# dohlee/chromoformer

Hardware: AMD Instinct MI355X
Metric: genes/sec training (bsz=64, default config) (higher is better)
Workload: dtype f32

## Files before the change

chromoformer_amd/_lib.py:

```python
from __future__ import annotations

import ctypes as C
import os
import subprocess

_HERE = os.path.dirname(os.path.abspath(__file__))
LIB_PATH = os.environ.get("CF_LIB_PATH") or os.path.join(_HERE, "libchromoformer_hip.so")
FLAGS_PATH = LIB_PATH + ".flags"
CSRC = os.path.join(_HERE, "csrc")
MAX_RES = 3
BUCKET_REG, BUCKET_PE = 1, 2
BUCKET_REG_HI, BUCKET_REG_LO = 4, 8
PART_REG_HI, PART_REG_LO = 8, 16


class cf_config(C.Structure):
    _fields_ = [
        ("n_feats", C.c_int), ("d_emb", C.c_int), ("d_head", C.c_int), ("n_out", C.c_int), ("n_res", C.c_int),
        ("binsizes", C.c_int * MAX_RES), ("n_bins", C.c_int * MAX_RES), ("i_max", C.c_int),
        ("embed_layers", C.c_int), ("embed_heads", C.c_int), ("embed_dmodel", C.c_int), ("embed_dff", C.c_int),
        ("pair_layers", C.c_int), ("pair_heads", C.c_int), ("pair_dmodel", C.c_int), ("pair_dff", C.c_int),
        ("reg_layers", C.c_int), ("reg_heads", C.c_int), ("reg_dmodel", C.c_int), ("reg_dff", C.c_int),
        ("max_batch", C.c_int),
    ]
# ... 105 lines not shown
    "cf_pcre_shapley": (C.c_int, [C.c_void_p, C.POINTER(cf_batch), C.c_void_p, C.c_void_p, C.c_void_p]),
    "cf_pcre_epistasis": (C.c_int, [C.c_void_p, C.POINTER(cf_batch), C.c_void_p, C.c_void_p, C.c_void_p]),
    "cf_integrated_gradients": (C.c_int, [C.c_void_p, C.POINTER(cf_batch), C.POINTER(cf_ig_opts), C.POINTER(cf_input_grads), C.c_void_p,
                                          C.c_void_p, C.c_void_p, C.c_void_p]),
    "cf_integrated_gradients_raw": (C.c_int, [C.c_void_p, C.POINTER(cf_batch), C.POINTER(cf_ig_opts), C.POINTER(cf_input_grads),
                                              C.POINTER(cf_input_grads), C.c_void_p, C.c_void_p, C.c_void_p, C.c_void_p]),
    "cf_perturbation_scan": (C.c_int, [C.c_void_p, C.POINTER(cf_batch), C.POINTER(cf_scan_opts), C.c_void_p, C.c_void_p]),
    "cf_adamw_step": (C.c_int, [C.c_void_p, C.c_float, C.c_float, C.c_float, C.c_float, C.c_float, C.c_longlong, C.c_void_p]),
    "cf_debug_copy": (C.c_int, [C.c_void_p, C.c_char_p, C.c_void_p, C.POINTER(C.c_longlong), C.c_void_p]),
    "cf_debug_names": (C.c_char_p, [C.c_void_p]),
    "cf_reduce_adamw_part": (C.c_int, [C.c_void_p, C.c_int, C.c_int, C.c_float, C.c_float, C.c_float, C.c_float, C.c_float, C.c_longlong, C.c_int,
                                       C.c_void_p]),
    "cf_reduce_opt_part": (C.c_int, [C.c_void_p, C.c_int, C.c_int, C.c_float, C.c_float, C.c_float, C.c_float, C.c_float, C.c_longlong, C.c_int,
                                     C.c_void_p]),
    "cf_rider_arm": (C.c_int, [C.c_void_p, C.c_float, C.c_float, C.c_float, C.c_float, C.c_float, C.c_longlong, C.c_int, C.c_int]),
    "cf_launch_counts": (C.c_int, [C.c_void_p, C.POINTER(C.c_int), C.POINTER(C.c_int), C.POINTER(C.c_int)]),
    "cf_op_linear": (C.c_int, [C.c_void_p, C.c_void_p, C.c_void_p, C.c_void_p, C.c_int, C.c_int, C.c_int, C.c_int, C.c_void_p]),
    "cf_op_wgrad": (C.c_int, [C.c_void_p, C.c_void_p, C.c_void_p, C.c_int, C.c_int, C.c_int, C.c_void_p]),
    "cf_op_dgrad": (C.c_int, [C.c_void_p, C.c_void_p, C.c_void_p, C.c_int, C.c_int, C.c_int, C.c_void_p]),
    "cf_bin_regions": (C.c_int, [C.c_void_p, C.c_int, C.c_int, C.c_int, C.c_int, C.c_void_p]),
    "cf_bin_regions_multi": (C.c_int, [C.c_void_p, C.c_int, C.c_int, C.c_int, C.POINTER(C.c_int), C.POINTER(C.c_int), C.c_int, C.c_void_p]),
    "cf_bin_regions_multi_backward": (C.c_int, [C.c_void_p, C.c_int, C.c_int, C.c_int, C.POINTER(C.c_int), C.POINTER(C.c_int), C.c_int, C.c_int,
                                                C.c_void_p]),
    "cf_embed_full": (C.c_int, [C.c_void_p, C.POINTER(cf_batch), C.POINTER(C.c_void_p), C.c_void_p]),
    "cf_gather_batch": (C.c_int, [C.c_void_p, C.POINTER(cf_store), C.c_void_p, C.c_void_p, C.POINTER(cf_batch), C.c_void_p, C.c_void_p]),
    "cf_gather_batch_fwd": (C.c_int, [C.c_void_p, C.POINTER(cf_store), C.c_void_p, C.c_void_p, C.POINTER(cf_batch), C.c_void_p, C.c_void_p]),
    "cf_gather_batch_next": (C.c_int, [C.c_void_p, C.POINTER(cf_store), C.c_void_p, C.c_void_p, C.POINTER(cf_batch), C.c_void_p, C.c_void_p]),
    "cf_gather_batch_only": (C.c_int, [C.c_void_p, C.POINTER(cf_store), C.c_void_p, C.c_void_p, C.POINTER(cf_batch), C.c_void_p, C.c_void_p]),
    "cf_record_step_bwd": (C.c_int, [C.c_void_p, C.c_void_p, C.c_void_p, C.c_void_p, C.c_void_p, C.c_int, C.c_void_p, C.c_void_p, C.c_void_p, C.c_void_p]),
    "cf_record_step": (C.c_int, [C.c_void_p, C.c_void_p, C.c_void_p, C.c_void_p, C.c_void_p, C.c_int, C.c_void_p, C.c_void_p, C.c_void_p, C.c_void_p]),
# ... 104 lines not shown
```

chromoformer_amd/csrc/cf_api.hip:

```cpp
#include "../../include/chromoformer_hip.h"
#include "cf_kernels.h"
#include "cf_input_grad.h"
#include "cf_attn_maps.h"
#include "cf_ablate.h"
#include "cf_coalition.h"
#include "cf_ig.h"
#include "cf_scan.h"
#include "cf_x0_gather.h"

#include <algorithm>
#include <cmath>
#include <cstdarg>
#include <cstdio>
#include <cstdlib>
#include <cstring>
#include <map>
#include <string>
#include <vector>

using namespace cf;

static thread_local std::string g_err;
static int fail(const char* fmt, ...) {
    char buf[512];
// ... 257 lines not shown
    std::vector<WsEntry> ws;
    std::map<std::string, int> ws_index;
    std::string ws_names;
    bool planning = true;
    float *pe[kMaxRes], *pet[kMaxRes];
    float *pe2[kMaxRes], *pet2[kMaxRes];
    bool attc2 = false;
    bool attc1 = true;
    int attc_cap = 64;
    int xcd_map = 1;
    int n_wg_r = 0, n_cs_r = 0;
    long long bucket_split = 0;
    long long bucket_split_hi = 0;
    int n_wg_hi = 0, n_cs_hi = 0;
    int n_wg_short = 0;
    float *featc[kMaxRes], *ex0[kMaxRes], *edx0[kMaxRes], *edout[kMaxRes];
    CentreBuf E[kMaxRes];
    float *xp0[kMaxRes], *dxp0[kMaxRes], *resid[kMaxRes];
    std::vector<CentreBuf> P[kMaxRes];
    std::vector<float*> Rx[kMaxRes], dRx[kMaxRes];
    std::vector<RegBuf> R[kMaxRes];
    float *hin, *h1, *logits, *dlogits, *dh1, *dhin, *loss, *loss_part, *tdbg;
    float* dfreq_part = nullptr;
    bool reg_dfreq_ok = false;
    bool ig_smem_ok = false;
    float* abl_stash[kMaxRes] = {};
    float* abl_freq = nullptr;
    uint8_t* abl_mask[kMaxRes] = {};
    void* abl_mem = nullptr;
    unsigned* coal_tab = nullptr;
// ... 195 lines not shown
            t.k0 = k0;
            t.toff = -1;
            out.push_back(t);
        }
}
static WgJob wg1(const float* A, int lda, const float* B, int ldb, int rpg, float* C, int ldc, int Nn, int Kk) {
    WgJob j;
    memset(&j, 0, sizeof j);
    j.seg[0] = WgSeg{A, B, lda, ldb, rpg};
    j.nseg = 1;
    j.C = C;
    j.ldc = ldc;
    j.Nn = Nn;
    j.Kk = Kk;
    return j;
}
static void push_cs(std::vector<CsTile>& out, const float* src, int ld, int ncols, int rpg, int div, float* dst, const float* src2 = nullptr) {
    for (int c0 = 0; c0 < ncols; c0 += 64) out.push_back(CsTile{src, dst, ld, ncols, c0, rpg, div, src2});
}
static void push_post_cs(std::vector<CsTile>& out, const cf_handle* h, const float* part, int dff, int rpg,
                         const std::string& att_pre, const std::string& ff_pre, int div = kTile) {
    const int kD = h->cfg.d_emb;
    const int pw = post_partial_width(dff, kD);
    push_cs(out, part + 0, pw, kD, rpg, div, h->G_(ff_pre + "ln.weight"));
    push_cs(out, part + kD, pw, kD, rpg, div, h->G_(ff_pre + "ln.bias"));
    push_cs(out, part + 2 * kD, pw, kD, rpg, div, h->G_(ff_pre + "l2.bias"));
    push_cs(out, part + 3 * kD, pw, dff, rpg, div, h->G_(ff_pre + "l1.bias"));
    push_cs(out, part + 3 * kD + dff, pw, kD, rpg, div, h->G_(att_pre + "ln.weight"));
    push_cs(out, part + 4 * kD + dff, pw, kD, rpg, div, h->G_(att_pre + "ln.bias"));
    push_cs(out, part + 5 * kD + dff, pw, kD, rpg, div, h->G_(att_pre + "ff.bias"));
// ... 131 lines not shown
                const float* xin = l == 0 ? b.xin : h->P[r][l - 1].out;
                float* gc = h->G_(lp + "self_att.c_att.weight");
                push_centre_wg(wg, h, b, xin, kD, S, c.pair_dff, h->G_(lp + "self_att.p_att.weight"), gc, gc + (size_t)kD * kD,
                               lp + "self_att.", lp + "ff.", c.pair_heads);
                if (h->trunk) push_post_cs(cs, h, b.partial, c.pair_dff, 1, lp + "self_att.", lp + "ff.", 1);
                else push_post_cs(cs, h, b.partial, c.pair_dff, S, lp + "self_att.", lp + "ff.");
            }
        }
        for (int l = 0; l < c.reg_layers; ++l) {
            std::vector<WgTile>& wgR = l >= c.reg_layers / 2 ? wgHi : wgLo;
            std::vector<CsTile>& csR = l >= c.reg_layers / 2 ? csHi : csLo;
            const std::string lp = fmt("regulation.%d.transformer.layers.%d.", bs, l);
            const RegBuf& b = h->R[r][l];
            const int dff = c.reg_dff;
            const int RDm = c.reg_dmodel, RW = 4 * RDm;
            if (l + 1 == c.reg_layers && h->reg_row0 && h->reg8) {
                float* ga = h->G_(lp + "self_att.att.weight");
                push_wg(wgShort, wg1(b.dqkvg, T * RW, h->Rx[r][l], T * kD, 1, ga, kD, RDm, kD));
                push_wg(wgR, wg1(b.dqkvg + RDm, RW, h->Rx[r][l], kD, T, ga + (size_t)RDm * kD, kD, 2 * RDm, kD));
                push_wg(wgShort, wg1(b.dqkvg + 3 * RDm, T * RW, h->Rx[r][l], T * kD, 1, ga + (size_t)3 * RDm * kD, kD, RDm, kD));
                push_wg(wgShort, wg1(b.dt1, T * kD, b.a, T * RDm, 1, h->G_(lp + "self_att.ff.weight"), RDm, kD, RDm));
                push_wg(wgShort, wg1(b.dpre1, T * dff, b.y1, T * kD, 1, h->G_(lp + "ff.l1.weight"), kD, dff, kD));
                push_wg(wgShort, wg1(b.dt2, T * kD, b.hdn, T * dff, 1, h->G_(lp + "ff.l2.weight"), dff, kD, dff));
            } else {
            push_wg(wgR, wg1(b.dqkvg, RW, h->Rx[r][l], kD, T, h->G_(lp + "self_att.att.weight"), kD, RW, kD));
            push_wg(wgR, wg1(b.dt1, kD, b.a, RDm, T, h->G_(lp + "self_att.ff.weight"), RDm, kD, RDm));
            push_wg(wgR, wg1(b.dpre1, dff, b.y1, kD, T, h->G_(lp + "ff.l1.weight"), kD, dff, kD));
            push_wg(wgR, wg1(b.dt2, kD, b.hdn, dff, T, h->G_(lp + "ff.l2.weight"), dff, kD, dff));
            }
            if (h->reg8) {
                const std::string ap = lp + "self_att.", fp = lp + "ff.";
                push_cs(csR, h->dRx[r][l + 1], kD, kD, T, 1, h->G_(fp + "ln.weight"), b.xh2);
                push_cs(csR, h->dRx[r][l + 1], kD, kD, T, 1, h->G_(fp + "ln.bias"));
                push_cs(csR, b.dt2, kD, kD, T, 1, h->G_(fp + "l2.bias"));
                push_cs(csR, b.dpre1, dff, dff, T, 1, h->G_(fp + "l1.bias"));
                push_cs(csR, b.dy1, kD, kD, T, 1, h->G_(ap + "ln.weight"), b.xh1);
                push_cs(csR, b.dy1, kD, kD, T, 1, h->G_(ap + "ln.bias"));
                push_cs(csR, b.dt1, kD, kD, T, 1, h->G_(ap + "ff.bias"));
            } else {
                push_post_cs(csR, h, b.partial, dff, T, lp + "self_att.", lp + "ff.");
            }
            push_cs(csR, b.dgam, c.reg_heads, c.reg_heads, 1, 1, h->G_(lp + "self_att.gamma_f"));
        }
    }
// ... 56 lines not shown
    wg.insert(wg.begin(), wgHi.begin(), wgHi.end());
    cs.insert(cs.begin(), csLo.begin(), csLo.end());
    cs.insert(cs.begin(), csHi.begin(), csHi.end());
    h->wg_flops_per_gene = 0.0;
    for (const WgTile& t : wg) {
        if (t.n0 || t.k0) continue;
        for (int sgi = 0; sgi < t.nseg; ++sgi) h->wg_flops_per_gene += 2.0 * t.seg[sgi].rows_per_gene * (double)t.Nn * t.Kk;
    }
    if (h->wg_tiles) (void)hipFree(h->wg_tiles);
    if (h->cs_tiles) (void)hipFree(h->cs_tiles);
    h->n_wg = (int)wg.size();
    h->n_cs = (int)cs.size();
    HIP_TRY(hipMalloc(&h->wg_tiles, wg.size() * sizeof(WgTile)));
    HIP_TRY(hipMalloc(&h->cs_tiles, cs.size() * sizeof(CsTile)));
    HIP_TRY(hipMemcpy(h->wg_tiles, wg.data(), wg.size() * sizeof(WgTile), hipMemcpyHostToDevice));
    HIP_TRY(hipMemcpy(h->cs_tiles, cs.data(), cs.size() * sizeof(CsTile), hipMemcpyHostToDevice));
    return 0;
}

extern "C" int cf_abi_version(void) { return CF_ABI_VERSION; }
extern "C" const char* cf_last_error(void) { return g_err.c_str(); }

extern "C" int cf_param_layout(const cf_config* cfg, cf_layout* layout, cf_param_desc* table, int cap) {
    if (!cfg || !layout) return fail("cf_param_layout: null argument");
    std::vector<PDesc> v;
    if (build_layout(*cfg, v, *layout)) return -1;
    if (table) {
        if (cap < (int)v.size()) return fail("cf_param_layout: table capacity %d < %d", cap, (int)v.size());
        for (size_t i = 0; i < v.size(); ++i) {
            cf_param_desc& d = table[i];
            memset(&d, 0, sizeof d);
            snprintf(d.name, sizeof d.name, "%s", v[i].name.c_str());
            d.ndim = v[i].ndim;
            d.shape[0] = v[i].shape[0];
            d.shape[1] = v[i].shape[1];
            d.offset = v[i].offset;
// ... 340 lines not shown
static CentreParams embed_params(const cf_handle* h, int r) {
    const std::string pre = fmt("embed.%d.", h->cfg.binsizes[r]), lp = pre + "transformer.layers.0.";
    const float* att = h->P_(lp + "self_att.att.weight");
    const size_t kD = h->cfg.d_emb;
    return centre_params(h, lp + "self_att.", lp + "ff.", att, att + (size_t)kD * kD, att + (size_t)2 * kD * kD,
                         h->P_(pre + "lin_proj.weight"));
}
static CentreParams pair_params(const cf_handle* h, int r, int l) {
    const std::string pre = fmt("pairwise_interaction.%d.", h->cfg.binsizes[r]), lp = pre + fmt("transformer.layers.%d.", l);
    const float* c_att = h->P_(lp + "self_att.c_att.weight");
    const size_t kD = h->cfg.d_emb;
    return centre_params(h, lp + "self_att.", lp + "ff.", h->P_(lp + "self_att.p_att.weight"), c_att, c_att + (size_t)kD * kD,
                         h->P_(pre + "lin_proj_pcre.weight"));
}

static const void* trunk_kernel(bool bwd, int dff_e, int dff_p, int pair_layers) {
    if (dff_e == 128 && dff_p == 256 && pair_layers == 2) return bwd ? (const void*)k_trunk_bwd<128, 256, 2> : (const void*)k_trunk_fwd<128, 256, 2>;
    return nullptr;
}
static void fill_centre_dev(CentreLayerDev& d, const CentreParams& p, const CentreBuf& b) {
    d.wq_t = p.wq_t, d.wk = p.wk, d.wv_t = p.wv_t, d.wo_t = p.wo_t, d.bo = p.bo, d.g1 = p.g1, d.be1 = p.be1;
    d.w1_t = p.w1_t, d.b1 = p.b1, d.w2_t = p.w2_t, d.b2 = p.b2, d.g2 = p.g2, d.be2 = p.be2;
    d.wq = p.wq, d.wk_t = p.wk_t, d.wv = p.wv, d.wo = p.wo, d.w1 = p.w1, d.w2 = p.w2;
    d.q = b.q, d.qt = b.qt, d.p = b.p, d.w = b.w, d.xbar = b.xbar, d.a = b.a, d.xh1 = b.xh1, d.rs1 = b.rs1, d.y1 = b.y1;
    d.hdn = b.hdn, d.xh2 = b.xh2, d.rs2 = b.rs2, d.out = b.out, d.xin = b.xin;
    d.dt2 = b.dt2, d.dpre1 = b.dpre1, d.dt1 = b.dt1, d.da = b.da, d.dxbar = b.dxbar, d.dqt = b.dqt, d.du = b.du, d.dq = b.dq;
    d.dx = b.dx, d.partial = b.partial;
}
static int build_trunk_table(cf_handle* h) {
    const cf_config& c = h->cfg;
    h->trunk = false;
    if (h->embed_dense || !h->attc2 || c.i_max > kAGMax || c.pair_layers > kMaxPairLayers || kPostWaves != 8) return 0;
    if (c.embed_heads != 2 || c.pair_heads != 2 || c.d_emb != kD) return 0;
    if (!trunk_kernel(false, c.embed_dff, c.pair_dff, c.pair_layers)) return 0;
    if (const char* e = getenv("CF_TRUNK"))
        if (atoi(e) == 0) return 0;
    size_t need = 0;
    for (int r = 0; r < c.n_res; ++r) need = std::max(need, trunk_smem(c.n_bins[r], c.n_feats, std::max(c.embed_dff, c.pair_dff)));
    if (need > 160 * 1024) return 0;
    const size_t need_bwd = std::max(need, (size_t)(kAT / 64) * kWgWaveLds * sizeof(float));
    if (need_bwd > 160 * 1024) return 0;
    if (hipFuncSetAttribute(trunk_kernel(false, c.embed_dff, c.pair_dff, c.pair_layers), hipFuncAttributeMaxDynamicSharedMemorySize, (int)need) != hipSuccess ||
        hipFuncSetAttribute(trunk_kernel(true, c.embed_dff, c.pair_dff, c.pair_layers), hipFuncAttributeMaxDynamicSharedMemorySize, (int)need_bwd) != hipSuccess)
        return 0;
    std::vector<TrunkResDev> tab(c.n_res);
    for (int r = 0; r < c.n_res; ++r) {
        TrunkResDev& t = tab[r];
        memset(&t, 0, sizeof t);
        fill_centre_dev(t.E, embed_params(h, r), h->E[r]);
        for (int l = 0; l < c.pair_layers; ++l) fill_centre_dev(t.P[l], pair_params(h, r, l), h->P[r][l]);
        t.pe = h->pe[r], t.pe2 = h->pe2[r], t.pet2 = h->pet2[r];
        t.wlp_e = embed_params(h, r).wlp;
        t.wlp_p = pair_params(h, r, 0).wlp;
        t.lin_p = h->P_(fmt("pairwise_interaction.%d.lin_proj_p.weight", c.binsizes[r]));
        t.lin_p_t = h->T_(fmt("pairwise_interaction.%d.lin_proj_p.weight", c.binsizes[r]));
// ... 723 lines not shown
            h->pend_record = false;
        }
        ta.lp_jobs = h->lp_jobs;
        ta.rd_tiles = nullptr;
        ta.rd_n = 0;
        ta.rd_batch = B;
        memset(&ta.rd_opt, 0, sizeof ta.rd_opt);
        const bool riding = h->rider.armed;
        if (riding) {
            if (h->capturing) return fail("cf_backward_part: armed riders carry this step's AdamW scalars as launch arguments and cannot be captured");
            ta.rd_n = std::min(h->rider.max_tiles, h->n_wg_r - h->n_wg_short);
            ta.rd_tiles = h->wg_tiles + h->n_wg_short;
            ta.rd_opt = h->rider.o;
        }
        void* kargs[] = {&ta};
        const size_t rider_lds = (size_t)(kAT / 64) * kWgWaveLds * sizeof(float);
        const int rider_rows = ta.rd_n > 0 ? (ta.rd_n + B * (kAT / 64) - 1) / (B * (kAT / 64)) : 0;
        h->time_mark("k_trunk_bwd", st);
        const hipError_t le = hipLaunchKernel(trunk_kernel(true, c.embed_dff, c.pair_dff, c.pair_layers), dim3(B, nres + rider_rows), dim3(kAT), kargs,
                                              ta.rd_n > 0 ? std::max(h->trunk_smem_bytes, rider_lds) : h->trunk_smem_bytes, st);
        h->time_mark("k_trunk_bwd", st);
        ++g_launches;
        if (le != hipSuccess || hipGetLastError() != hipSuccess) {
            return fail("launch k_trunk_bwd failed: %s", hipGetErrorString(le));
        }
        if (riding) {
            h->rider.armed = false;
            h->rider.done = ta.rd_n;
        }
        return 0;
    }
// ... 906 lines not shown
```

chromoformer_amd/csrc/cf_kernels.h:

```cpp
#pragma once
#include <hip/hip_runtime.h>
#include <stdint.h>
#include <type_traits>
#ifndef CF_TRUNK_NT
#define CF_TRUNK_NT 0
#endif

#ifndef CF_TID_OPAQUE
#define CF_TID_OPAQUE 1
#endif
#if CF_TID_OPAQUE
namespace cf {
struct TidProxy {
    struct X {
        __device__ __forceinline__ operator unsigned() const {
            unsigned t = __builtin_amdgcn_workitem_id_x();
            asm volatile("" : "+v"(t));
            return t;
        }
    } x;
    struct Y { __device__ __forceinline__ operator unsigned() const { return __builtin_amdgcn_workitem_id_y(); } } y;
    struct Z { __device__ __forceinline__ operator unsigned() const { return __builtin_amdgcn_workitem_id_z(); } } z;
};
}
// ... 1693 lines not shown
#define CF_OPT_NT 1
#endif
#ifndef CF_RIDER_NT
#define CF_RIDER_NT 0
#endif
#ifndef CF_WG_M
#define CF_WG_M 32
#endif
constexpr int kWgM = CF_WG_M;
constexpr int kWgTk = CF_WG_TK;
constexpr int kWgLdA = 64 + 16;
constexpr int kWgLdB = kWgTk + 4;
__device__ __forceinline__ float4 f4_keep_if(bool keep, const float4& v) {
    return make_float4(keep ? v.x : 0.f, keep ? v.y : 0.f, keep ? v.z : 0.f, keep ? v.w : 0.f);
}
__device__ __forceinline__ bool wg_tile_interior(const WgTile& t) {
    bool ok = t.n0 + 64 <= t.Nn && t.k0 + kWgTk <= t.Kk;
    for (int s = 0; s < t.nseg; ++s) {
        const WgSeg& sg = t.seg[s];
        ok = ok && ((sg.lda | sg.ldb | t.n0 | t.k0) & 3) == 0 && ((reinterpret_cast<uintptr_t>(sg.A) | reinterpret_cast<uintptr_t>(sg.B)) & 15) == 0;
    }
    return ok;
}
template <bool OPT, int D = 1>
__device__ __forceinline__ void wgrad_tile_impl(const WgTile& t, int batch, const AdamFuse* o, float (*As)[kWgM * kWgLdA], float (*Bs)[kWgM * kWgLdB],
                                                const int tid) {
    constexpr int NH = kWgTk / 64;
    const int w = tid >> 6, lane = tid & 63, lr = lane & 15, lq = lane >> 4;
    const int kc = t.k0 + 4 * lr;
    f32x4 acc[4 * NH];
    zero_acc(acc);
// ... 97 lines not shown
                    if (CF_OPT_NT) stg4_nt(o->p + off, pp[i]); else stg4(o->p + off, pp[i]);
                    if (CF_OPT_NT) stg4_nt(o->m + off, mm[i]); else stg4(o->m + off, mm[i]);
                    if (CF_OPT_NT) stg4_nt(o->v + off, vv[i]); else stg4(o->v + off, vv[i]);
                    if (o->keep_grads) stg4(cp, g4);
                    if (o->tiled && t.toff >= 0) {
                        const int ra = t.trow0 + row, k = kc + 64 * h;
                        stg4(o->tiled + t.toff + ((size_t)(ra >> 4) * (t.ldc >> 4) + (k >> 4)) * 256 + (((k & 15) >> 2) * 16 + (ra & 15)) * 4, pp[i]);
                    }
                } else {
                    stg4(cp, g4);
                }
            }
        }
    }
}
constexpr int kWgWaveLds = kWgM * kWgLdA + kWgM * kWgLdB;
template <bool OPT>
__device__ __forceinline__ void wgrad_tile_wave(const WgTile& t, int batch, const AdamFuse* o, float* lds, unsigned long long* stamp = nullptr) {
    static_assert(kWgTk == 64, "one 64 x 64 tile per wave");
    const int lane = threadIdx.x & 63, lr = lane & 15, lq = lane >> 4;
    float* As = lds;
    float* Bs = lds + kWgM * kWgLdA;
    const int kc = t.k0 + 4 * lr;
    f32x4 acc[4][4];
#pragma unroll
    for (int rt = 0; rt < 4; ++rt) zero_acc(acc[rt]);
    const int sm = lane >> 4, sc = (lane & 15) * 4;
    constexpr int NP = kWgM / 4;
    const bool interior = wg_tile_interior(t);
    auto run = [&](auto fast_c) {
        constexpr bool FAST = decltype(fast_c)::value;
        for (int s = 0; s < t.nseg; ++s) {
            const WgSeg sg = t.seg[s];
            const int M = sg.rows_per_gene * batch, nst = (M + kWgM - 1) / kWgM;
            const bool va = ((sg.lda | t.n0) & 3) == 0 && (reinterpret_cast<uintptr_t>(sg.A) & 15) == 0;
            const bool vb = ((sg.ldb | t.k0) & 3) == 0 && (reinterpret_cast<uintptr_t>(sg.B) & 15) == 0;
            float4 ra[NP], rb[NP];
            auto fetch = [&](int st) {
// ... 38 lines not shown
                    for (int rt = 0; rt < 4; ++rt) {
                        const float av = ap[4 * i * kWgLdA + 16 * rt];
                        acc[rt][0] = mfma4(av, bv.x, acc[rt][0]);
                        acc[rt][1] = mfma4(av, bv.y, acc[rt][1]);
                        acc[rt][2] = mfma4(av, bv.z, acc[rt][2]);
                        acc[rt][3] = mfma4(av, bv.w, acc[rt][3]);
                    }
                }
            }
        }
    };
    if (stamp) stamp[0] = __builtin_amdgcn_s_memtime();
    if (interior) run(std::true_type{});
    else run(std::false_type{});
    if (stamp) stamp[1] = __builtin_amdgcn_s_memtime();
    if (kc >= t.Kk) return;
#pragma unroll
    for (int rt = 0; rt < 4; ++rt) {
        float4 pp[4], mm[4], vv[4];
        if (OPT) {
#pragma unroll
            for (int i = 0; i < 4; ++i) {
                const int row = min(t.n0 + rt * 16 + lq * 4 + i, t.Nn - 1);
                const size_t off = (size_t)(t.C + (size_t)row * t.ldc + kc - o->gbase);
                pp[i] = CF_RIDER_NT ? ldg4_nt(o->p + off) : ldg4(o->p + off);
                mm[i] = CF_RIDER_NT ? ldg4_nt(o->m + off) : ldg4(o->m + off);
                vv[i] = CF_RIDER_NT ? ldg4_nt(o->v + off) : ldg4(o->v + off);
            }
            __builtin_amdgcn_sched_barrier(0);
        }
#pragma unroll
        for (int i = 0; i < 4; ++i) {
            const int row = t.n0 + rt * 16 + lq * 4 + i;
            if (row < t.Nn) {
                float* cp = t.C + (size_t)row * t.ldc + kc;
                const float4 g4 = make_float4(acc[rt][0][i], acc[rt][1][i], acc[rt][2][i], acc[rt][3][i]);
                if (OPT) {
                    const size_t off = (size_t)(cp - o->gbase);
                    adamw_elem(pp[i].x, g4.x, mm[i].x, vv[i].x, *o);
                    adamw_elem(pp[i].y, g4.y, mm[i].y, vv[i].y, *o);
                    adamw_elem(pp[i].z, g4.z, mm[i].z, vv[i].z, *o);
                    adamw_elem(pp[i].w, g4.w, mm[i].w, vv[i].w, *o);
                    if (CF_RIDER_NT) stg4_nt(o->p + off, pp[i]); else stg4(o->p + off, pp[i]);
                    if (CF_RIDER_NT) stg4_nt(o->m + off, mm[i]); else stg4(o->m + off, mm[i]);
                    if (CF_RIDER_NT) stg4_nt(o->v + off, vv[i]); else stg4(o->v + off, vv[i]);
                    if (o->keep_grads) stg4(cp, g4);
                } else {
                    stg4(cp, g4);
                }
            }
        }
    }
}
template <bool OPT = false>
__device__ __forceinline__ void wgrad_tile(const WgTile& t, int batch, const AdamFuse* o = nullptr) {
    __shared__ __attribute__((aligned(16))) float As[1][kWgM * kWgLdA];
    __shared__ __attribute__((aligned(16))) float Bs[1][kWgM * kWgLdB];
    wgrad_tile_impl<OPT>(t, batch, o, As, Bs, threadIdx.x);
}

__device__ __forceinline__ int xcd_tile(int b, int n, int on) {
    const int per = (n + 7) >> 3;
    return on ? (b & 7) * per + (b >> 3) : b;
}
__host__ __device__ inline int xcd_grid(int n) { return 8 * ((n + 7) >> 3); }
__global__ __launch_bounds__(256) void k_wgrad(const WgTile* __restrict__ tiles, int n, int batch, int xcd) {
    const int t = xcd_tile(blockIdx.x, n, xcd);
// ... 275 lines not shown
```

chromoformer_amd/csrc/cf_trunk.h:

```cpp
#pragma once

namespace cf {

constexpr int kMaxPairLayers = 4;

struct CentreLayerDev {
    const float *wq_t, *wk, *wv_t, *wo_t, *bo, *g1, *be1, *w1_t, *b1, *w2_t, *b2, *g2, *be2;
    const float *wq, *wk_t, *wv, *wo, *w1, *w2;
    float *q, *qt, *p, *w, *xbar, *a, *xh1, *rs1, *y1, *hdn, *xh2, *rs2, *out, *xin;
    float *dt2, *dpre1, *dt1, *da, *dxbar, *dqt, *du, *dq, *dx, *partial;
};
struct TrunkResDev {
    CentreLayerDev E, P[kMaxPairLayers];
    const float *pe, *pe2, *pet2;
    const float *wlp_e, *wlp_p;
    const float *lin_p_t, *lin_p;
    float *ex0, *featc, *xp0, *dxp0, *edout, *rx0, *drx0;
    float *lp_part_e, *lp_part_p;
    int L, Lpad, LT, pad_;
};
struct TrunkArgs {
    const TrunkResDev* tab;
    const float* pfeats[kMaxRes];
    const uint8_t* pmask[kMaxRes];
// ... 378 lines not shown
    float* const p1 = ldc(&J[1].partial);
    float* out = (job ? p1 : p0) + (size_t)g * (kD * F) + e * F;
#pragma unroll
    for (int k = 0; k < 4; ++k)
        if (fh * 4 + k < F) stg(out + fh * 4 + k, acc[k]);
}

template <int DFF_E, int DFF_P, int PL>
__global__ __launch_bounds__(kAT) void k_trunk_bwd(TrunkArgs a) {
    extern __shared__ __attribute__((aligned(16))) float smem[];
    if ((int)blockIdx.y >= a.n_res) {
        const int w = threadIdx.x >> 6;
        const int t = (((int)blockIdx.y - a.n_res) * gridDim.x + blockIdx.x) * (kAT / 64) + w;
        unsigned long long* stamp = a.tdbg && blockIdx.x == 0 && (int)blockIdx.y == a.n_res && (threadIdx.x & 63) == 0 ? a.tdbg + 64 + 4 * w : nullptr;
        if (stamp) stamp[3] = __builtin_amdgcn_s_memtime();
        if (t < a.rd_n) wgrad_tile_wave<true>(a.rd_tiles[t], a.rd_batch, &a.rd_opt, smem + w * kWgWaveLds, stamp);
        if (stamp) {
            asm volatile("s_waitcnt vmcnt(0)" ::: "memory");
            stamp[2] = __builtin_amdgcn_s_memtime();
        }
        return;
    }
    if (a.rec.cursor && blockIdx.x == 0 && blockIdx.y == 0) record_block(a.rec);
    const int r = a.n_res - 1 - (int)blockIdx.y;
    const TrunkResDev* R = a.tab + r;
    constexpr int DFF_MAX = DFF_E > DFF_P ? DFF_E : DFF_P;
    float* sm = smem;
    float* persist = smem + trunk_scratch_floats(TF(L), DFF_MAX);
    TrunkCtx c{R, a.cfeats[r], a.cmask[r], a.cmstride[r], (int)blockIdx.x, a.S, a.T, a.F, 1, a.scale, a.rscale};
    int stamp_i = 32;
    if (a.tdbg && blockIdx.x == 0 && blockIdx.y == CF_STAMP_Y && threadIdx.x == 0) a.tdbg[stamp_i++] = __builtin_amdgcn_s_memtime();
// ... 37 lines not shown
```

include/chromoformer_hip.h:

```cpp
#ifndef CHROMOFORMER_HIP_H
#define CHROMOFORMER_HIP_H

#include <stddef.h>
#include <stdint.h>

#ifdef __cplusplus
extern "C" {
#endif

#define CF_MAX_RES 3
#define CF_ABI_VERSION 1

typedef struct cf_config {
    int n_feats;
    int d_emb;
    int d_head;
    int n_out;
    int n_res;
    int binsizes[CF_MAX_RES];
    int n_bins[CF_MAX_RES];
    int i_max;
    int embed_layers, embed_heads, embed_dmodel, embed_dff;
    int pair_layers, pair_heads, pair_dmodel, pair_dff;
    int reg_layers, reg_heads, reg_dmodel, reg_dff;
// ... 115 lines not shown
int cf_graph_launch(cf_handle* h, int graph_id, void* stream);

int cf_timing_select(cf_handle* h, const char* kernel);
int cf_timing_read(cf_handle* h, float* total_ms, int* count);
double cf_wgrad_flops(cf_handle* h, int B);
double cf_kernel_flops(cf_handle* h, const char* kernel, int B);
int cf_cu_count(cf_handle* h);
int cf_debug_copy(cf_handle* h, const char* name, float* dst, long long* n_floats, void* stream);
const char* cf_debug_names(cf_handle* h);
int cf_reduce_adamw_part(cf_handle* h, int B, int reduce_buckets, float lr, float beta1, float beta2, float eps,
                         float weight_decay, long long step, int adam_buckets, void* stream);
int cf_reduce_opt_part(cf_handle* h, int B, int bucket, float lr, float beta1, float beta2, float eps, float weight_decay,
                       long long step, int keep_grads, void* stream);
int cf_rider_arm(cf_handle* h, float lr, float beta1, float beta2, float eps, float weight_decay, long long step, int keep_grads,
                 int max_tiles);
int cf_launch_counts(cf_handle* h, int* fwd, int* bwd, int* opt);

int cf_op_linear(const float* A, const float* W, const float* bias, float* C, int M, int N, int K,
                 int relu, void* stream);
int cf_op_wgrad(const float* dY, const float* X, float* dW, int M, int N, int K, void* stream);
int cf_op_dgrad(const float* dY, const float* W, float* dX, int M, int N, int K, void* stream);

typedef struct cf_dense_layer {
    const float *wq, *wkv;
    const float *wo, *bo, *ln1_g, *ln1_b;
    const float *w1, *b1, *w2, *b2, *ln2_g, *ln2_b;
    int d_ff;
} cf_dense_layer;
long long cf_op_dense_layer_workspace(int N, int Lq, int Lk, int d_ff);
int cf_op_dense_layer_fwd(const cf_dense_layer* w, const float* x_q, const float* x_kv, const unsigned char* qvalid,
// ... 105 lines not shown
```

Before: 131,300.

## Share operand panels across eight rider wgrad tiles in one workgroup

Rider weight-gradient tiles in the trunk backward kernel used to run one wave per tile, each staging its own A/B operands in private LDS. When a group of eight consecutive tiles writes the same output matrix with the same segments and sits within a 4x4 panel rectangle, the whole workgroup now cooperatively stages shared A and B panels into double-buffered LDS and each wave computes its tile from them. This cuts redundant global operand loads, at the cost of a larger LDS reservation for the backward kernel and added workgroup-wide synchronisation. A host query, cf_rider_groups, reports how many groups qualify.

Result: no change. 131,100 (-0.2%).

```diff
diff --git a/chromoformer_amd/_lib.py b/chromoformer_amd/_lib.py
--- a/chromoformer_amd/_lib.py
+++ b/chromoformer_amd/_lib.py
@@ -143,6 +143,7 @@
     "cf_reduce_opt_part": (C.c_int, [C.c_void_p, C.c_int, C.c_int, C.c_float, C.c_float, C.c_float, C.c_float, C.c_float, C.c_longlong, C.c_int,
                                      C.c_void_p]),
     "cf_rider_arm": (C.c_int, [C.c_void_p, C.c_float, C.c_float, C.c_float, C.c_float, C.c_float, C.c_longlong, C.c_int, C.c_int]),
+    "cf_rider_groups": (C.c_int, [C.c_void_p, C.POINTER(cf_config), C.c_int, C.c_int, C.POINTER(C.c_int), C.POINTER(C.c_int)]),
     "cf_launch_counts": (C.c_int, [C.c_void_p, C.POINTER(C.c_int), C.POINTER(C.c_int), C.POINTER(C.c_int)]),
     "cf_op_linear": (C.c_int, [C.c_void_p, C.c_void_p, C.c_void_p, C.c_void_p, C.c_int, C.c_int, C.c_int, C.c_int, C.c_void_p]),
     "cf_op_wgrad": (C.c_int, [C.c_void_p, C.c_void_p, C.c_void_p, C.c_int, C.c_int, C.c_int, C.c_void_p]),
diff --git a/chromoformer_amd/csrc/cf_api.hip b/chromoformer_amd/csrc/cf_api.hip
--- a/chromoformer_amd/csrc/cf_api.hip
+++ b/chromoformer_amd/csrc/cf_api.hip
@@ -295,6 +295,7 @@
     long long bucket_split_hi = 0;
     int n_wg_hi = 0, n_cs_hi = 0;
     int n_wg_short = 0;
+    std::vector<WgTile> wg_r_host;
     float *featc[kMaxRes], *ex0[kMaxRes], *edx0[kMaxRes], *edout[kMaxRes];
     CentreBuf E[kMaxRes];
     float *xp0[kMaxRes], *dxp0[kMaxRes], *resid[kMaxRes];
@@ -520,6 +521,27 @@
     j.Nn = Nn;
     j.Kk = Kk;
     return j;
+}
+struct RegWgSrc {
+    const float *dqkvg, *dt1, *a, *dpre1, *y1, *dt2, *hdn, *x;
+    float *g_att, *g_ff, *g_l1, *g_l2;
+};
+static void push_reg_layer_wg(std::vector<WgTile>& wgShort, std::vector<WgTile>& wgR, const cf_config& c, const RegWgSrc& b, bool row0_last) {
+    const int kD = c.d_emb, T = c.i_max + 1, dff = c.reg_dff, RDm = c.reg_dmodel, RW = 4 * RDm;
+    if (row0_last) {
+        float* ga = b.g_att;
+        push_wg(wgShort, wg1(b.dqkvg, T * RW, b.x, T * kD, 1, ga, kD, RDm, kD));
+        push_wg(wgR, wg1(b.dqkvg + RDm, RW, b.x, kD, T, ga + (size_t)RDm * kD, kD, 2 * RDm, kD));
+        push_wg(wgShort, wg1(b.dqkvg + 3 * RDm, T * RW, b.x, T * kD, 1, ga + (size_t)3 * RDm * kD, kD, RDm, kD));
+        push_wg(wgShort, wg1(b.dt1, T * kD, b.a, T * RDm, 1, b.g_ff, RDm, kD, RDm));
+        push_wg(wgShort, wg1(b.dpre1, T * dff, b.y1, T * kD, 1, b.g_l1, kD, dff, kD));
+        push_wg(wgShort, wg1(b.dt2, T * kD, b.hdn, T * dff, 1, b.g_l2, dff, kD, dff));
+    } else {
+        push_wg(wgR, wg1(b.dqkvg, RW, b.x, kD, T, b.g_att, kD, RW, kD));
+        push_wg(wgR, wg1(b.dt1, kD, b.a, RDm, T, b.g_ff, RDm, kD, RDm));
+        push_wg(wgR, wg1(b.dpre1, dff, b.y1, kD, T, b.g_l1, kD, dff, kD));
+        push_wg(wgR, wg1(b.dt2, kD, b.hdn, dff, T, b.g_l2, dff, kD, dff));
+    }
 }
 static void push_cs(std::vector<CsTile>& out, const float* src, int ld, int ncols, int rpg, int div, float* dst, const float* src2 = nullptr) {
     for (int c0 = 0; c0 < ncols; c0 += 64) out.push_back(CsTile{src, dst, ld, ncols, c0, rpg, div, src2});
@@ -681,20 +703,9 @@
             const RegBuf& b = h->R[r][l];
             const int dff = c.reg_dff;
             const int RDm = c.reg_dmodel, RW = 4 * RDm;
-            if (l + 1 == c.reg_layers && h->reg_row0 && h->reg8) {
-                float* ga = h->G_(lp + "self_att.att.weight");
-                push_wg(wgShort, wg1(b.dqkvg, T * RW, h->Rx[r][l], T * kD, 1, ga, kD, RDm, kD));
-                push_wg(wgR, wg1(b.dqkvg + RDm, RW, h->Rx[r][l], kD, T, ga + (size_t)RDm * kD, kD, 2 * RDm, kD));
-                push_wg(wgShort, wg1(b.dqkvg + 3 * RDm, T * RW, h->Rx[r][l], T * kD, 1, ga + (size_t)3 * RDm * kD, kD, RDm, kD));
-                push_wg(wgShort, wg1(b.dt1, T * kD, b.a, T * RDm, 1, h->G_(lp + "self_att.ff.weight"), RDm, kD, RDm));
-                push_wg(wgShort, wg1(b.dpre1, T * dff, b.y1, T * kD, 1, h->G_(lp + "ff.l1.weight"), kD, dff, kD));
-                push_wg(wgShort, wg1(b.dt2, T * kD, b.hdn, T * dff, 1, h->G_(lp + "ff.l2.weight"), dff, kD, dff));
-            } else {
-            push_wg(wgR, wg1(b.dqkvg, RW, h->Rx[r][l], kD, T, h->G_(lp + "self_att.att.weight"), kD, RW, kD));
-            push_wg(wgR, wg1(b.dt1, kD, b.a, RDm, T, h->G_(lp + "self_att.ff.weight"), RDm, kD, RDm));
-            push_wg(wgR, wg1(b.dpre1, dff, b.y1, kD, T, h->G_(lp + "ff.l1.weight"), kD, dff, kD));
-            push_wg(wgR, wg1(b.dt2, kD, b.hdn, dff, T, h->G_(lp + "ff.l2.weight"), dff, kD, dff));
-            }
+            const RegWgSrc src{b.dqkvg, b.dt1, b.a, b.dpre1, b.y1, b.dt2, b.hdn, h->Rx[r][l], h->G_(lp + "self_att.att.weight"),
+                               h->G_(lp + "self_att.ff.weight"), h->G_(lp + "ff.l1.weight"), h->G_(lp + "ff.l2.weight")};
+            push_reg_layer_wg(wgShort, wgR, c, src, l + 1 == c.reg_layers && h->reg_row0 && h->reg8);
             if (h->reg8) {
                 const std::string ap = lp + "self_att.", fp = lp + "ff.";
                 push_cs(csR, h->dRx[r][l + 1], kD, kD, T, 1, h->G_(fp + "ln.weight"), b.xh2);
@@ -781,12 +792,48 @@
     HIP_TRY(hipMalloc(&h->wg_tiles, wg.size() * sizeof(WgTile)));
     HIP_TRY(hipMalloc(&h->cs_tiles, cs.size() * sizeof(CsTile)));
     HIP_TRY(hipMemcpy(h->wg_tiles, wg.data(), wg.size() * sizeof(WgTile), hipMemcpyHostToDevice));
+    h->wg_r_host.assign(wg.begin(), wg.begin() + h->n_wg_r);
     HIP_TRY(hipMemcpy(h->cs_tiles, cs.data(), cs.size() * sizeof(CsTile), hipMemcpyHostToDevice));
     return 0;
 }
 
 extern "C" int cf_abi_version(void) { return CF_ABI_VERSION; }
 extern "C" const char* cf_last_error(void) { return g_err.c_str(); }
+
+extern "C" int cf_rider_groups(cf_handle* h, const cf_config* cfg, int row0_last, int max_tiles, int* n_groups, int* n_shared) {
+    if (!n_groups || !n_shared || (!h && !cfg)) return fail("cf_rider_groups: null argument");
+    std::vector<WgTile> synth;
+    const WgTile* win = nullptr;
+    int avail = 0;
+    if (h) {
+        if ((int)h->wg_r_host.size() != h->n_wg_r) return fail("cf_rider_groups: the gradient tables have not been built");
+        win = h->wg_r_host.data() + h->n_wg_short;
+        avail = h->n_wg_r - h->n_wg_short;
+    } else {
+        const cf_config& c = *cfg;
+        if (c.n_res < 1 || c.n_res > kMaxRes || c.reg_layers < 1 || c.i_max < 1) return fail("cf_rider_groups: bad configuration");
+        std::vector<WgTile> hi, lo, sh;
+        uintptr_t next = 1u << 24;
+        auto arr = [&]() { next += (uintptr_t)1 << 24; return reinterpret_cast<float*>(next); };
+        for (int r = 0; r < c.n_res; ++r)
+            for (int l = 0; l < c.reg_layers; ++l) {
+                const RegWgSrc src{arr(), arr(), arr(), arr(), arr(), arr(), arr(), arr(), arr(), arr(), arr(), arr()};
+                push_reg_layer_wg(sh, l >= c.reg_layers / 2 ? hi : lo, c, src, row0_last != 0 && l + 1 == c.reg_layers);
+            }
+        synth = hi;
+        synth.insert(synth.end(), lo.begin(), lo.end());
+        win = synth.data();
+        avail = (int)synth.size();
+    }
+    const int n = std::max(0, std::min(max_tiles, avail));
+    *n_groups = (n + kWgGroup - 1) / kWgGroup;
+    *n_shared = 0;
+    for (int g0 = 0; g0 < n; g0 += kWgGroup) {
+        WgGroup g;
+        if (CF_RIDER_GROUPS && wg_group_rect(win + g0, std::min(kWgGroup, n - g0), g)) ++*n_shared;
+    }
+    return 0;
+}
 
 extern "C" int cf_param_layout(const cf_config* cfg, cf_layout* layout, cf_param_desc* table, int cap) {
     if (!cfg || !layout) return fail("cf_param_layout: null argument");
@@ -1157,6 +1204,7 @@
                          h->P_(pre + "lin_proj_pcre.weight"));
 }
 
+static size_t rider_lds_bytes() { return sizeof(float) * (size_t)std::max((kAT / 64) * kWgWaveLds, CF_RIDER_GROUPS ? kWgGroupLds : 0); }
 static const void* trunk_kernel(bool bwd, int dff_e, int dff_p, int pair_layers) {
     if (dff_e == 128 && dff_p == 256 && pair_layers == 2) return bwd ? (const void*)k_trunk_bwd<128, 256, 2> : (const void*)k_trunk_fwd<128, 256, 2>;
     return nullptr;
@@ -1181,7 +1229,7 @@
     size_t need = 0;
     for (int r = 0; r < c.n_res; ++r) need = std::max(need, trunk_smem(c.n_bins[r], c.n_feats, std::max(c.embed_dff, c.pair_dff)));
     if (need > 160 * 1024) return 0;
-    const size_t need_bwd = std::max(need, (size_t)(kAT / 64) * kWgWaveLds * sizeof(float));
+    const size_t need_bwd = std::max(need, rider_lds_bytes());
     if (need_bwd > 160 * 1024) return 0;
     if (hipFuncSetAttribute(trunk_kernel(false, c.embed_dff, c.pair_dff, c.pair_layers), hipFuncAttributeMaxDynamicSharedMemorySize, (int)need) != hipSuccess ||
         hipFuncSetAttribute(trunk_kernel(true, c.embed_dff, c.pair_dff, c.pair_layers), hipFuncAttributeMaxDynamicSharedMemorySize, (int)need_bwd) != hipSuccess)
@@ -1935,7 +1983,7 @@
             ta.rd_opt = h->rider.o;
         }
         void* kargs[] = {&ta};
-        const size_t rider_lds = (size_t)(kAT / 64) * kWgWaveLds * sizeof(float);
+        const size_t rider_lds = rider_lds_bytes();
         const int rider_rows = ta.rd_n > 0 ? (ta.rd_n + B * (kAT / 64) - 1) / (B * (kAT / 64)) : 0;
         h->time_mark("k_trunk_bwd", st);
         const hipError_t le = hipLaunchKernel(trunk_kernel(true, c.embed_dff, c.pair_dff, c.pair_layers), dim3(B, nres + rider_rows), dim3(kAT), kargs,
diff --git a/chromoformer_amd/csrc/cf_kernels.h b/chromoformer_amd/csrc/cf_kernels.h
--- a/chromoformer_amd/csrc/cf_kernels.h
+++ b/chromoformer_amd/csrc/cf_kernels.h
@@ -1731,7 +1731,7 @@
 __device__ __forceinline__ float4 f4_keep_if(bool keep, const float4& v) {
     return make_float4(keep ? v.x : 0.f, keep ? v.y : 0.f, keep ? v.z : 0.f, keep ? v.w : 0.f);
 }
-__device__ __forceinline__ bool wg_tile_interior(const WgTile& t) {
+__host__ __device__ __forceinline__ bool wg_tile_interior(const WgTile& t) {
     bool ok = t.n0 + 64 <= t.Nn && t.k0 + kWgTk <= t.Kk;
     for (int s = 0; s < t.nseg; ++s) {
         const WgSeg& sg = t.seg[s];
@@ -1859,6 +1859,48 @@
         }
     }
 }
+template <bool OPT>
+__device__ __forceinline__ void wgrad_wave_store(const WgTile& t, f32x4 (&acc)[4][4], const AdamFuse* o) {
+    const int lane = threadIdx.x & 63, lr = lane & 15, lq = lane >> 4;
+    const int kc = t.k0 + 4 * lr;
+    if (kc >= t.Kk) return;
+#pragma unroll
+    for (int rt = 0; rt < 4; ++rt) {
+        float4 pp[4], mm[4], vv[4];
+        if (OPT) {
+#pragma unroll
+            for (int i = 0; i < 4; ++i) {
+                const int row = min(t.n0 + rt * 16 + lq * 4 + i, t.Nn - 1);
+                const size_t off = (size_t)(t.C + (size_t)row * t.ldc + kc - o->gbase);
+                pp[i] = CF_RIDER_NT ? ldg4_nt(o->p + off) : ldg4(o->p + off);
+                mm[i] = CF_RIDER_NT ? ldg4_nt(o->m + off) : ldg4(o->m + off);
+                vv[i] = CF_RIDER_NT ? ldg4_nt(o->v + off) : ldg4(o->v + off);
+            }
+            __builtin_amdgcn_sched_barrier(0);
+        }
+#pragma unroll
+        for (int i = 0; i < 4; ++i) {
+            const int row = t.n0 + rt * 16 + lq * 4 + i;
+            if (row < t.Nn) {
+                float* cp = t.C + (size_t)row * t.ldc + kc;
+                const float4 g4 = make_float4(acc[rt][0][i], acc[rt][1][i], acc[rt][2][i], acc[rt][3][i]);
+                if (OPT) {
+                    const size_t off = (size_t)(cp - o->gbase);
+                    adamw_elem(pp[i].x, g4.x, mm[i].x, vv[i].x, *o);
+                    adamw_elem(pp[i].y, g4.y, mm[i].y, vv[i].y, *o);
+                    adamw_elem(pp[i].z, g4.z, mm[i].z, vv[i].z, *o);
+                    adamw_elem(pp[i].w, g4.w, mm[i].w, vv[i].w, *o);
+                    if (CF_RIDER_NT) stg4_nt(o->p + off, pp[i]); else stg4(o->p + off, pp[i]);
+                    if (CF_RIDER_NT) stg4_nt(o->m + off, mm[i]); else stg4(o->m + off, mm[i]);
+                    if (CF_RIDER_NT) stg4_nt(o->v + off, vv[i]); else stg4(o->v + off, vv[i]);
+                    if (o->keep_grads) stg4(cp, g4);
+                } else {
+                    stg4(cp, g4);
+                }
+            }
+        }
+    }
+}
 constexpr int kWgWaveLds = kWgM * kWgLdA + kWgM * kWgLdB;
 template <bool OPT>
 __device__ __forceinline__ void wgrad_tile_wave(const WgTile& t, int batch, const AdamFuse* o, float* lds, unsigned long long* stamp = nullptr) {
@@ -1866,7 +1908,6 @@
     const int lane = threadIdx.x & 63, lr = lane & 15, lq = lane >> 4;
     float* As = lds;
     float* Bs = lds + kWgM * kWgLdA;
-    const int kc = t.k0 + 4 * lr;
     f32x4 acc[4][4];
 #pragma unroll
     for (int rt = 0; rt < 4; ++rt) zero_acc(acc[rt]);
@@ -1935,43 +1976,130 @@
     if (interior) run(std::true_type{});
     else run(std::false_type{});
     if (stamp) stamp[1] = __builtin_amdgcn_s_memtime();
-    if (kc >= t.Kk) return;
-#pragma unroll
-    for (int rt = 0; rt < 4; ++rt) {
-        float4 pp[4], mm[4], vv[4];
-        if (OPT) {
-#pragma unroll
-            for (int i = 0; i < 4; ++i) {
-                const int row = min(t.n0 + rt * 16 + lq * 4 + i, t.Nn - 1);
-                const size_t off = (size_t)(t.C + (size_t)row * t.ldc + kc - o->gbase);
-                pp[i] = CF_RIDER_NT ? ldg4_nt(o->p + off) : ldg4(o->p + off);
-                mm[i] = CF_RIDER_NT ? ldg4_nt(o->m + off) : ldg4(o->m + off);
-                vv[i] = CF_RIDER_NT ? ldg4_nt(o->v + off) : ldg4(o->v + off);
-            }
+    wgrad_wave_store<OPT>(t, acc, o);
+}
+#ifndef CF_RIDER_GROUPS
+#define CF_RIDER_GROUPS 1
+#endif
+constexpr int kWgGroup = 8;
+constexpr int kWgGroupPanels = 4;
+struct WgGroup {
+    int nmin, kmin, na, nb;
+};
+__host__ __device__ __forceinline__ bool wg_group_entry_ok(const WgTile& u, const WgTile& f) {
+    bool same = (u.nseg == f.nseg) & (u.C == f.C) & (u.ldc == f.ldc) & (u.Nn == f.Nn) & (u.Kk == f.Kk);
+#pragma unroll
+    for (int s = 0; s < 4; ++s)
+        same = same & (u.seg[s].A == f.seg[s].A) & (u.seg[s].B == f.seg[s].B) & (u.seg[s].lda == f.seg[s].lda) & (u.seg[s].ldb == f.seg[s].ldb) &
+               (u.seg[s].rows_per_gene == f.seg[s].rows_per_gene);
+    bool interior = (u.n0 + 64 <= u.Nn) & (u.k0 + kWgTk <= u.Kk);
+#pragma unroll
+    for (int s = 0; s < 4; ++s)
+        interior = interior & ((s >= u.nseg) | ((((u.seg[s].lda | u.seg[s].ldb | u.n0 | u.k0) & 3) == 0) &
+                                                 (((reinterpret_cast<uintptr_t>(u.seg[s].A) | reinterpret_cast<uintptr_t>(u.seg[s].B)) & 15) == 0)));
+    return same & interior & (((u.n0 - f.n0) & 63) == 0) & (((u.k0 - f.k0) & 63) == 0) & (u.nseg >= 1) & (u.nseg <= 4);
+}
+__host__ __device__ __forceinline__ bool wg_group_span_ok(int nlo, int nhi, int klo, int khi, WgGroup& g) {
+    g.nmin = nlo, g.kmin = klo, g.na = (nhi - nlo) / 64 + 1, g.nb = (khi - klo) / 64 + 1;
+    return g.na <= kWgGroupPanels && g.nb <= kWgGroupPanels;
+}
+inline bool wg_group_rect(const WgTile* t, int live, WgGroup& g) {
+    if (live < 1 || live > kWgGroup || kWgTk != 64) return false;
+    int nlo = t[0].n0, nhi = t[0].n0, klo = t[0].k0, khi = t[0].k0;
+    bool ok = true;
+    for (int j = 0; j < live; ++j) {
+        ok = ok && wg_group_entry_ok(t[j], t[0]);
+        nlo = std::min(nlo, t[j].n0), nhi = std::max(nhi, t[j].n0), klo = std::min(klo, t[j].k0), khi = std::max(khi, t[j].k0);
+    }
+    return wg_group_span_ok(nlo, nhi, klo, khi, g) && ok;
+}
+__device__ __forceinline__ bool wg_group_rect_wave(const WgTile* t, int live, WgGroup& g) {
+    if (live < 1 || live > kWgGroup || kWgTk != 64) return false;
+    const int j = min((int)(threadIdx.x & 63), live - 1);
+    const WgTile& u = t[j];
+    const bool ok = wg_group_entry_ok(u, t[0]);
+    int nlo = __builtin_amdgcn_readlane(u.n0, 0), nhi = nlo, klo = __builtin_amdgcn_readlane(u.k0, 0), khi = klo;
+#pragma unroll
+    for (int q = 1; q < kWgGroup; ++q) {
+        const int n = __builtin_amdgcn_readlane(u.n0, q), k = __builtin_amdgcn_readlane(u.k0, q);
+        nlo = min(nlo, n), nhi = max(nhi, n), klo = min(klo, k), khi = max(khi, k);
+    }
+    const bool all_ok = __builtin_amdgcn_ballot_w64(!ok) == 0;
+    return wg_group_span_ok(nlo, nhi, klo, khi, g) && all_ok;
+}
+constexpr int kWgGroupBuf = kWgGroupPanels * kWgM * (kWgLdA + kWgLdB);
+constexpr int kWgGroupLds = 2 * kWgGroupBuf;
+template <bool OPT>
+__device__ __forceinline__ void wgrad_group8(const WgTile* tiles, int live, const WgGroup g, int batch, const AdamFuse* o, float* lds, unsigned long long* stamp = nullptr) {
+    static_assert(kWgTk == 64 && kWgM * 16 == 512, "a stage of a panel is one float4 per thread of a 512-thread workgroup");
+    const int tid = threadIdx.x, lane = tid & 63, lr = lane & 15, lq = lane >> 4;
+    const int w = __builtin_amdgcn_readfirstlane(tid >> 6);
+    const bool mine = w < live;
+    const WgTile& t = tiles[mine ? w : 0];
+    const WgTile& f = tiles[0];
+    const int pa = (t.n0 - g.nmin) >> 6, pb = (t.k0 - g.kmin) >> 6;
+    f32x4 acc[4][4];
+#pragma unroll
+    for (int rt = 0; rt < 4; ++rt) zero_acc(acc[rt]);
+    const int sm = tid >> 4, sc = (tid & 15) * 4;
+    constexpr int kPanA = kWgM * kWgLdA, kPanB = kWgM * kWgLdB, kOffB = kWgGroupPanels * kPanA;
+    if (stamp) stamp[0] = __builtin_amdgcn_s_memtime();
+    for (int s = 0; s < f.nseg; ++s) {
+        const WgSeg sg = f.seg[s];
+        const int M = sg.rows_per_gene * batch, nst = (M + kWgM - 1) / kWgM;
+        float4 ra[kWgGroupPanels], rb[kWgGroupPanels];
+        auto fetch = [&](int st) {
+            const int mc = min(st * kWgM + sm, M - 1);
+            const float* ap = sg.A + (size_t)mc * sg.lda + g.nmin + sc;
+            const float* bp = sg.B + (size_t)mc * sg.ldb + g.kmin + sc;
+#pragma unroll
+            for (int p = 0; p < kWgGroupPanels; ++p) {
+                if (p < g.na) ra[p] = CF_RIDER_OPND_NT ? ldg4_nt(ap + 64 * p) : ldg4(ap + 64 * p);
+                if (p < g.nb) rb[p] = CF_RIDER_OPND_NT ? ldg4_nt(bp + 64 * p) : ldg4(bp + 64 * p);
+            }
+        };
+        auto put = [&](int st) {
+            float* buf = lds + (st & 1) * kWgGroupBuf;
+            const bool keep = st * kWgM + sm < M;
+#pragma unroll
+            for (int p = 0; p < kWgGroupPanels; ++p) {
+                if (p < g.na) *reinterpret_cast<float4*>(&buf[p * kPanA + sm * kWgLdA + sc]) = f4_keep_if(keep, ra[p]);
+                if (p < g.nb) *reinterpret_cast<float4*>(&buf[kOffB + p * kPanB + sm * kWgLdB + sc]) = f4_keep_if(keep, rb[p]);
+            }
+        };
+        if (s > 0) __syncthreads();
+        if (nst > 0) {
+            fetch(0);
+            put(0);
+        }
+        for (int st = 0; st < nst; ++st) {
+            __syncthreads();
             __builtin_amdgcn_sched_barrier(0);
-        }
-#pragma unroll
-        for (int i = 0; i < 4; ++i) {
-            const int row = t.n0 + rt * 16 + lq * 4 + i;
-            if (row < t.Nn) {
-                float* cp = t.C + (size_t)row * t.ldc + kc;
-                const float4 g4 = make_float4(acc[rt][0][i], acc[rt][1][i], acc[rt][2][i], acc[rt][3][i]);
-                if (OPT) {
-                    const size_t off = (size_t)(cp - o->gbase);
-                    adamw_elem(pp[i].x, g4.x, mm[i].x, vv[i].x, *o);
-                    adamw_elem(pp[i].y, g4.y, mm[i].y, vv[i].y, *o);
-                    adamw_elem(pp[i].z, g4.z, mm[i].z, vv[i].z, *o);
-                    adamw_elem(pp[i].w, g4.w, mm[i].w, vv[i].w, *o);
-                    if (CF_RIDER_NT) stg4_nt(o->p + off, pp[i]); else stg4(o->p + off, pp[i]);
-                    if (CF_RIDER_NT) stg4_nt(o->m + off, mm[i]); else stg4(o->m + off, mm[i]);
-                    if (CF_RIDER_NT) stg4_nt(o->v + off, vv[i]); else stg4(o->v + off, vv[i]);
-                    if (o->keep_grads) stg4(cp, g4);
-                } else {
-                    stg4(cp, g4);
+            if (st + 1 < nst) fetch(st + 1);
+            __builtin_amdgcn_sched_barrier(0);
+            const float* buf = lds + (st & 1) * kWgGroupBuf;
+            const float* ap = &buf[pa * kPanA + lq * kWgLdA + lr];
+            const float* bp = &buf[kOffB + pb * kPanB + lq * kWgLdB + 4 * lr];
+            if (mine) {
+#pragma unroll
+                for (int i = 0; i < kWgM / 4; ++i) {
+                    const float4 bv = *reinterpret_cast<const float4*>(bp + 4 * i * kWgLdB);
+#pragma unroll
+                    for (int rt = 0; rt < 4; ++rt) {
+                        const float av = ap[4 * i * kWgLdA + 16 * rt];
+                        acc[rt][0] = mfma4(av, bv.x, acc[rt][0]);
+                        acc[rt][1] = mfma4(av, bv.y, acc[rt][1]);
+                        acc[rt][2] = mfma4(av, bv.z, acc[rt][2]);
+                        acc[rt][3] = mfma4(av, bv.w, acc[rt][3]);
+                    }
                 }
             }
-        }
-    }
+            __builtin_amdgcn_sched_barrier(0);
+            if (st + 1 < nst) put(st + 1);
+        }
+    }
+    if (stamp) stamp[1] = __builtin_amdgcn_s_memtime();
+    if (mine) wgrad_wave_store<OPT>(t, acc, o);
 }
 template <bool OPT = false>
 __device__ __forceinline__ void wgrad_tile(const WgTile& t, int batch, const AdamFuse* o = nullptr) {
diff --git a/chromoformer_amd/csrc/cf_trunk.h b/chromoformer_amd/csrc/cf_trunk.h
--- a/chromoformer_amd/csrc/cf_trunk.h
+++ b/chromoformer_amd/csrc/cf_trunk.h
@@ -416,7 +416,11 @@
         const int t = (((int)blockIdx.y - a.n_res) * gridDim.x + blockIdx.x) * (kAT / 64) + w;
         unsigned long long* stamp = a.tdbg && blockIdx.x == 0 && (int)blockIdx.y == a.n_res && (threadIdx.x & 63) == 0 ? a.tdbg + 64 + 4 * w : nullptr;
         if (stamp) stamp[3] = __builtin_amdgcn_s_memtime();
-        if (t < a.rd_n) wgrad_tile_wave<true>(a.rd_tiles[t], a.rd_batch, &a.rd_opt, smem + w * kWgWaveLds, stamp);
+        const int g0 = t - w, live = min(kWgGroup, a.rd_n - g0);
+        WgGroup grp;
+        if (CF_RIDER_GROUPS && live > 0 && wg_group_rect_wave(a.rd_tiles + g0, live, grp))
+            wgrad_group8<true>(a.rd_tiles + g0, live, grp, a.rd_batch, &a.rd_opt, smem, stamp);
+        else if (t < a.rd_n) wgrad_tile_wave<true>(a.rd_tiles[t], a.rd_batch, &a.rd_opt, smem + w * kWgWaveLds, stamp);
         if (stamp) {
             asm volatile("s_waitcnt vmcnt(0)" ::: "memory");
             stamp[2] = __builtin_amdgcn_s_memtime();
diff --git a/include/chromoformer_hip.h b/include/chromoformer_hip.h
--- a/include/chromoformer_hip.h
+++ b/include/chromoformer_hip.h
@@ -153,6 +153,7 @@
                        long long step, int keep_grads, void* stream);
 int cf_rider_arm(cf_handle* h, float lr, float beta1, float beta2, float eps, float weight_decay, long long step, int keep_grads,
                  int max_tiles);
+int cf_rider_groups(cf_handle* h, const cf_config* cfg, int row0_last, int max_tiles, int* n_groups, int* n_shared);
 int cf_launch_counts(cf_handle* h, int* fwd, int* bwd, int* opt);
 
 int cf_op_linear(const float* A, const float* W, const float* bias, float* C, int M, int N, int K,
```
